# renmengye/rec-attend-public

Hardware: AMD Instinct MI355X
Metric: instance-timesteps/sec, full_model forward 512x512 T=16 (whole job; pipelined throughput: 8 batches in flight per GPU, fill and drain of the pipeline inside the timed region; config.lone_batch_* = one sync-bracketed forward) (higher is better)
Workload: dtype f32; 1 GPU; cfg2: CVPPP-arch full_model eval forward, 512x512, T=16, B=8 per GPU, y_out+s_out; arch=cvppp, H=512, W=512, T=16, batch_per_gpu=8, global_batch=8, parallelism=batch-sharded x1, no collective, ranks_in_communicator=1, hip_graph=True, tile_tickets=False, batches_in_flight=8, pipeline_slots=4, batches_per_launch=2, input=resident in HBM, output=left in HBM

## Files before the change

### rec-attend-public_amd/csrc/ra_common.h

```cpp
#pragma once
#include <hip/hip_runtime.h>

#include <cstdarg>
#include <cstdio>
#include <cstdlib>

#include "recattend.h"

namespace ra {

void set_error(const char *fmt, ...);

inline hipStream_t as_stream(void *s) { return reinterpret_cast<hipStream_t>(s); }

inline int launch_status(const char *what) {
  hipError_t e = hipGetLastError();
  if (e != hipSuccess) {
    set_error("%s: %s", what, hipGetErrorString(e));
    return static_cast<int>(e);
  }
  return 0;
}

inline int fail(int code, const char *fmt, ...) {
  char buf[256];
  va_list ap;
  va_start(ap, fmt);
  vsnprintf(buf, sizeof(buf), fmt, ap);
  va_end(ap);
  set_error("%s", buf);
  return code;
}

constexpr int kWave = 64;

inline int env_int(const char *name, int dflt) {
  const char *e = getenv(name);
  return e ? atoi(e) : dflt;
}

struct [[maybe_unused]] MaxDynamicLds {
  template <typename K>
  MaxDynamicLds(K kern, size_t bytes) {
    (void)hipFuncSetAttribute(reinterpret_cast<const void *>(kern), hipFuncAttributeMaxDynamicSharedMemorySize, (int)bytes);
  }
};

inline int cu_count() {
  static const int n = [] {
    int dev = 0;
    hipDeviceProp_t prop;
    if (hipGetDevice(&dev) == hipSuccess && hipGetDeviceProperties(&prop, dev) == hipSuccess && prop.multiProcessorCount > 0)
      return (int)prop.multiProcessorCount;
    return 256;
  }();
  return n;
}
template <typename K>
int wgs_per_cu(K kern, size_t lds) {
  MaxDynamicLds{kern, lds};
  int n = 0;
  if (hipOccupancyMaxActiveBlocksPerMultiprocessor(&n, kern, 256, lds) != hipSuccess || n < 1) n = 1;
  return n;
}

int tail_prio(int kind = 4);
__device__ __forceinline__ void raise_prio(int p) {
  if (p >= 3) __builtin_amdgcn_s_setprio(3);
  else if (p == 2) __builtin_amdgcn_s_setprio(2);
  else if (p == 1) __builtin_amdgcn_s_setprio(1);
}

constexpr int kTicketPoolStride = 32;
constexpr int kTicketSlotWords = 8 * kTicketPoolStride;
constexpr int kTicketMinTilesPerWg = 3;
unsigned *take_ticket_slots(int n, int grid_x);
int xcc_census_ok();

__device__ __forceinline__ int xcc_id() {
  unsigned id;
  asm volatile("s_getreg_b32 %0, hwreg(HW_REG_XCC_ID)" : "=s"(id));
  return (int)(id & 7u);
}
__device__ __forceinline__ unsigned ticket_draw(unsigned *pool) {
  const __amdgpu_buffer_rsrc_t r = __builtin_amdgcn_make_buffer_rsrc(pool, 0, 4, 0x00020000);
  return (unsigned)__builtin_amdgcn_raw_ptr_buffer_atomic_add_i32(1, r, 0, 0, 1);
}
struct TicketWalk {
  unsigned *pool;
  int base, lim;
  int cur, nxt;
  unsigned pend;
  __device__ __forceinline__ int tile_of(unsigned t) const { return t < (unsigned)lim ? base + (int)t : -1; }
  unsigned t0, t1;
  __device__ __forceinline__ void issue(unsigned *slot, int ntiles) {
    const int x = xcc_id(), chunk = (ntiles + 7) >> 3;
    pool = slot + x * kTicketPoolStride;
    base = x * chunk;
    lim = base + chunk <= ntiles ? chunk : (ntiles > base ? ntiles - base : 0);
    t0 = t1 = 0;
    if (threadIdx.x == 0) {
      t0 = ticket_draw(pool);
      t1 = ticket_draw(pool);
    }
  }
  __device__ __forceinline__ void begin(volatile unsigned *sh) {
    if (threadIdx.x == 0) sh[1] = t0;
    __syncthreads();
    cur = tile_of(__builtin_amdgcn_readfirstlane(sh[1]));
    nxt = -1;
    pend = t1;
  }
  __device__ __forceinline__ void request() {
    if (threadIdx.x == 0) pend = ticket_draw(pool);
  }
  __device__ __forceinline__ void read_next(volatile unsigned *sh) { nxt = tile_of(__builtin_amdgcn_readfirstlane(sh[0])); }
  __device__ __forceinline__ void publish(volatile unsigned *sh) {
    if (threadIdx.x == 0) sh[0] = pend;
  }
  __device__ __forceinline__ void step() { cur = nxt; }
};

__host__ __device__ inline int ceil_div(int a, int b) { return (a + b - 1) / b; }
__host__ __device__ inline int round_up(int a, int b) { return ceil_div(a, b) * b; }

inline void plan_walk(int *plan, int ntiles, int grid, int xcd_map) {
  int lo = ntiles / grid, hi = ceil_div(ntiles, grid);
  if (xcd_map) {
    const int chunk = (ntiles + 7) >> 3, nwx = grid >> 3;
    lo = hi = 0;
    for (int x = 0; x < 8; ++x) {
      const int n = x * chunk >= ntiles ? 0 : (x * chunk + chunk < ntiles ? chunk : ntiles - x * chunk);
      lo = (x == 0 || n / nwx < lo) ? n / nwx : lo;
      hi = ceil_div(n, nwx) > hi ? ceil_div(n, nwx) : hi;
    }
  }
  plan[RA_PLAN_GRID] = grid, plan[RA_PLAN_NTILES] = ntiles, plan[RA_PLAN_XCD_MAP] = xcd_map;
  plan[RA_PLAN_TILES_MIN] = lo, plan[RA_PLAN_TILES_MAX] = hi;
}
inline bool plan_have_device() {
  int n = 0;
  return hipGetDeviceCount(&n) == hipSuccess && n > 0;
}

}
```

### rec-attend-public_amd/csrc/ra_conv_pair.hip

```cpp
#include <cstdlib>

#include "ra_common.h"
#include "ra_split3.h"

namespace ra {
namespace cpair {

struct PArgs {
  const float *src;
  float *y;
  const float *wpA, *scA, *shA, *wpB, *scB, *shB;
  int C0, Hs, Ws, H, W, ups;
  int CoutAP, CoutB, CoutBP, poolB, Ho, Wo, reluA, reluB;
  const float *plane;
  int plane_chan;
  int bytes0, bytes_p;
  const float *cache;
  int cache_rows, cache_gx, bytes_c;
  int bytes_y;
  int xcd_map;
  float *rider_dst;
  int rider_quads;
  float rider_val;
  unsigned *tickets;
};

template <int CINA, int CMID, int NCB, int GX, int GYB>
struct PGeo {
  static constexpr int NCA = (CMID + 15) / 16;
  static constexpr int TWB = 8 * GX, THB = 8 * GYB, PMB = GX * GYB;
  static constexpr int GXA = GX + 1, GRA = THB / 2 + 1, NGA = GXA * GRA;
  static constexpr int AW = 8 * GXA, AH = 2 * GRA;
  static constexpr int LWA = AW + 2, LHA = AH + 2;
  static constexpr int NCGA = CINA / 4, CKA = CINA < 16 ? CINA : 16, NCHA = CINA / CKA, NCGAC = CKA / 4;
  static constexpr int NCGB = CMID / 4, CKB = CMID < 16 ? CMID : 16, NCHB = CMID / CKB, NCGBC = CKB / 4;
  static constexpr int KSA = 9 * NCGAC, KSB = 9 * NCGBC;
  static constexpr int IN_FLOATS = LHA * LWA * CINA;
  static constexpr int MID_FLOATS = AH * AW * CMID;
  static constexpr int RA = 4;
  static constexpr int GPW = (NGA + 3) / 4;
  static constexpr int ROUNDS = (GPW + RA - 1) / RA;
};

template <int N>
struct vec_of {
  typedef float type __attribute__((ext_vector_type(N)));
};

template <int CINA, int CMID, int NCB, int GX, int GYB>
__global__ __launch_bounds__(256) void conv_pair_mfma(const PArgs a, int tiles_x, int tiles_y) {
  using G = PGeo<CINA, CMID, NCB, GX, GYB>;
  constexpr int NCA = G::NCA;
  extern __shared__ __attribute__((aligned(16))) float lds[];
  float *tin = lds;
  float *tmid = lds + G::IN_FLOATS;
  typedef typename vec_of<G::NCGAC>::type avecA;
  typedef typename vec_of<G::NCGBC>::type avecB;

  const int tid = threadIdx.x, lane = tid & 63;
  const int wave = __builtin_amdgcn_readfirstlane(tid >> 6);
  const int m = lane & 15, ksub = lane >> 4;
  const int q = m >> 2, dy = (m >> 1) & 1, dx = m & 1;
  const int co_lane = lane & 15, qo = lane >> 4;
  const int per = tiles_x * tiles_y;
  const int b = blockIdx.x / per;
  const int trem = blockIdx.x - b * per;
  const int ty0 = (trem / tiles_x) * G::THB, tx0 = (trem % tiles_x) * G::TWB;

  {
    const int sy0 = a.ups ? (ty0 >> 1) : ty0, sx0 = a.ups ? (tx0 >> 1) : tx0;
    const float *base = a.src + ((size_t)(b * a.Hs + sy0) * a.Ws + sx0) * a.C0;
    for (int e = tid; e < G::LHA * G::LWA; e += 256) {
      const int rr = e / G::LWA - 2, cc = e % G::LWA - 2;
      const int Y = ty0 + rr, X = tx0 + cc;
      bool ok = (Y >= 0) & (Y < a.H) & (X >= 0) & (X < a.W);
      int ys = rr, xs = cc;
      if (a.ups) {
        ok = ok & (rr & 1) & (cc & 1);
        ys = rr >> 1;
        xs = cc >> 1;
      }
      f32x4 v[G::NCGA];
#pragma unroll
      for (int cg = 0; cg < G::NCGA; ++cg) {
        v[cg] = f32x4{0.f, 0.f, 0.f, 0.f};
        if (ok) v[cg] = *reinterpret_cast<const f32x4 *>(base + (ys * a.Ws + xs) * a.C0 + 4 * cg);
      }
      if (a.plane && ok) {
        const float pv = a.plane[(size_t)(b * a.Hs + sy0 + ys) * a.Ws + sx0 + xs];
        const int pg = a.plane_chan >> 2, slot = a.plane_chan & 3;
#pragma unroll
        for (int cg = 0; cg < G::NCGA; ++cg) {
          v[cg].x = (cg == pg && slot == 0) ? pv : v[cg].x;
          v[cg].y = (cg == pg && slot == 1) ? pv : v[cg].y;
          v[cg].z = (cg == pg && slot == 2) ? pv : v[cg].z;
          v[cg].w = (cg == pg && slot == 3) ? pv : v[cg].w;
        }
      }
      float *rec = tin + e * CINA;
#pragma unroll
      for (int ks = 0; ks < 4; ++ks) {
        if constexpr (G::NCGA == 1) {
          rec[ks] = v[0][ks];
// ... 347 lines not shown
    const int wrow0 = ty0 + wave * 2 * GYB, lcol0 = tx0 + 2 * qo;
#pragma unroll
    for (int n = 0; n < NCB; ++n) {
      const int co = 16 * n + co_lane;
      const float sc = a.scB[co], sh = a.shB[co];
      const bool co_ok = co < a.CoutB;
      const int obase = ((b * a.Ho + wrow0 / opool) * a.Wo + lcol0 / opool) * a.CoutB + co;
#pragma unroll
      for (int g = 0; g < G::PMB; ++g) {
        const int gx = g % GX, gy = g / GX;
        const int row0 = wrow0 + 2 * gy, col0 = lcol0 + 8 * gx;
        float v[4];
#pragma unroll
        for (int r = 0; r < 4; ++r) v[r] = fmaxf(acc[g][n][r] * sc + sh, loB);
        if (opool == 2) {
          const float o = fmaxf(fmaxf(v[0], v[1]), fmaxf(v[2], v[3]));
          if (co_ok && (row0 >> 1) < a.Ho && (col0 >> 1) < a.Wo)
            a.y[obase + (gy * a.Wo + 4 * gx) * a.CoutB] = o;
        } else {
#pragma unroll
          for (int r = 0; r < 4; ++r)
            if (co_ok && row0 + (r >> 1) < a.Ho && col0 + (r & 1) < a.Wo)
              a.y[obase + ((2 * gy + (r >> 1)) * a.Wo + 8 * gx + (r & 1)) * a.CoutB] = v[r];
        }
      }
    }
  }
  }
}

template <int CINA>
struct NGeo {
  static constexpr int TH = 16, TW = 32;
  static constexpr int NCGA = CINA / 4;
  static constexpr int AGX = 5, AGY = 5, NGA = AGX * AGY, GPW = (NGA + 3) / 4;
  static constexpr int AW = 41, AHS = TH + 2;
  static constexpr int LW = 43, LH = 4 * AGY + 2;
  static constexpr int LHL = TH + 4, LWL = TW + 6;
  static constexpr int IN_FLOATS = LH * LW * CINA;
  static constexpr int MID_FLOATS = AHS * AW * 8;
};

#ifndef RA_PAIR8_CACHE_AHEAD
#define RA_PAIR8_CACHE_AHEAD 0
#endif
#ifndef RA_PAIR8_OCC
#define RA_PAIR8_OCC 3
#endif
#ifdef RA_PROBE8
__device__ long long *ra_probe8_buf;
#define RA_PHASE_PROBE_BUF ra_probe8_buf
#define RA_PHASE_PROBE_WG blockIdx.x
#endif
#include "ra_phase_probe.h"
#ifdef RA_P8_NOBAR
#define RA_P8_SYNC() __builtin_amdgcn_s_waitcnt(0xc07f)
#else
#define RA_P8_SYNC() __syncthreads()
#endif
template <int CINA, bool CACHED, bool SPLIT = false>
__global__ __launch_bounds__(256, CACHED ? (SPLIT ? (RA_PAIR8_CACHE_AHEAD ? 2 : 3) : 4) : RA_PAIR8_OCC) void conv_pair8_mfma(const PArgs a, int tiles_x, int tiles_y, int ntiles) {
  using G = NGeo<CINA>;
  constexpr int NCGA = G::NCGA;
  static_assert(!CACHED || CINA == 4, "cached form: 4 input channels");
  static_assert(!SPLIT || CACHED, "the split-precision layer B exists for the cached (steady-state) form");
  constexpr int PLANE_B = G::AHS * G::AW * 16;
  constexpr int MIDF = SPLIT ? 3 * PLANE_B / 4 : G::MID_FLOATS;
  constexpr int RECA = CACHED ? 1 : CINA;
  extern __shared__ __attribute__((aligned(16))) float lds[];
  constexpr int IN_FLOATS = (G::LH * G::LW * RECA + 3) & ~3;
  float *tin = lds;
  float *tmid = lds + IN_FLOATS;
  typedef typename vec_of<NCGA>::type avecA;

  const int tid = threadIdx.x, lane = tid & 63;
  __shared__ unsigned tk_sh[2];
  TicketWalk tk;
  const bool dyn = a.tickets != nullptr;
  if (dyn) tk.issue(a.tickets, ntiles);
  const int wave = __builtin_amdgcn_readfirstlane(tid >> 6);
  const int m = lane & 15, ksub = lane >> 4;
  const int n = lane & 15, qo = lane >> 4;
  const int p = n >> 3, co = n & 7;
  const int per = tiles_x * tiles_y;

  const float scA = a.scA[co], scB = a.scB[co], shB = a.shB[co];
  const float loA = a.reluA ? 0.f : -__builtin_inff(), loB = a.reluB ? 0.f : -__builtin_inff();
  const int qA = m >> 2, rA = m & 3, pA = ksub >> 1, coA0 = 4 * (ksub & 1);
  f32x4 scA4, shA4;
#pragma unroll
  for (int j = 0; j < 4; ++j) scA4[j] = a.scA[coA0 + j], shA4[j] = a.shA[coA0 + j];
  const bool fill = !CACHED && a.cache != nullptr;
  float bA[CACHED ? 1 : 12][NCGA], bB[12][2];
  float bAc[3];
#pragma unroll
  for (int ky = 0; ky < 3; ++ky) {
    const int kx = ksub - p;
    const bool ok = (kx >= 0) & (kx <= 2);
    const int tap = ok ? ky * 3 + kx : 0;
    const float w = a.wpA[((tap * NCGA + (a.plane_chan >> 2)) * 4 + (a.plane_chan & 3)) * a.CoutAP + co];
    bAc[ky] = (CACHED && ok) ? w * scA : 0.f;
  }
#pragma unroll
  for (int ky = 0; ky < 3; ++ky)
#pragma unroll
    for (int kxp = 0; kxp < 4; ++kxp) {
      const int kx = kxp - p;
      const bool ok = (kx >= 0) & (kx <= 2);
      const int tap = ok ? ky * 3 + kx : 0;
      if constexpr (!CACHED) {
#pragma unroll
        for (int cg = 0; cg < NCGA; ++cg) {
          const float w = a.wpA[((tap * NCGA + cg) * 4 + ksub) * a.CoutAP + co];
          bA[ky * 4 + kxp][cg] = ok ? w * (fill ? 1.f : scA) : 0.f;
        }
      }
#pragma unroll
      for (int cg = 0; cg < 2; ++cg) {
        const float w = a.wpB[((tap * 2 + cg) * 4 + ksub) * a.CoutBP + co];
        bB[ky * 4 + kxp][cg] = ok ? w * scB : 0.f;
      }
    }

  s16x8 wB[SPLIT ? 3 : 1][SPLIT ? 3 : 1];
  if constexpr (SPLIT) {
#pragma unroll
    for (int ky = 0; ky < 3; ++ky) {
      const int kx = ksub - p;
      const bool ok = (kx >= 0) & (kx <= 2);
      const int tap = ok ? ky * 3 + kx : 0;
#pragma unroll
      for (int j = 0; j < 8; j += 2) {
        const float w0 = a.wpB[((tap * 2 + (j >> 2)) * 4 + (j & 3)) * a.CoutBP + co];
        const float w1 = a.wpB[((tap * 2 + ((j + 1) >> 2)) * 4 + ((j + 1) & 3)) * a.CoutBP + co];
        unsigned H, M, L;
        split3_pair(ok ? w0 * scB : 0.f, ok ? w1 * scB : 0.f, H, M, L);
        wB[ky][0][j] = (short)(H & 0xffffu), wB[ky][0][j + 1] = (short)(H >> 16);
        wB[ky][1][j] = (short)(M & 0xffffu), wB[ky][1][j + 1] = (short)(M >> 16);
        wB[ky][2][j] = (short)(L & 0xffffu), wB[ky][2][j + 1] = (short)(L >> 16);
      }
    }
  }
  const __amdgpu_buffer_rsrc_t rs = __builtin_amdgcn_make_buffer_rsrc(const_cast<float *>(a.src), 0, a.bytes0, 0x00020000);
  const __amdgpu_buffer_rsrc_t rp = __builtin_amdgcn_make_buffer_rsrc(
      const_cast<float *>(a.plane ? a.plane : a.src), 0, a.plane ? a.bytes_p : 0, 0x00020000);
  constexpr int NE = G::LHL * G::LWL, NIT = (NE + 255) / 256;
  int e_rr[NIT], e_cc[NIT];
#pragma unroll
  for (int i = 0; i < NIT; ++i) {
    const int e = tid + 256 * i;
    e_rr[i] = e / G::LWL;
    e_cc[i] = e - e_rr[i] * G::LWL;
    if (e >= NE) e_rr[i] = -(1 << 20);
  }
  unsigned e_offp[NIT], e_offs[NIT];
#pragma unroll
  for (int i = 0; i < NIT; ++i) {
    const bool in = tid + 256 * i < NE;
    const unsigned o = (unsigned)(e_rr[i] * a.W + e_cc[i]) * 4u;
    e_offp[i] = in ? o : 0x80000000u;
    e_offs[i] = in ? o * CINA : 0x80000000u;
  }
  struct TC {
    int b, ty, tx;
  };
  auto split = [&](int t) {
    TC c;
    c.b = t / per;
    const int r = t - c.b * per;
    c.ty = r / tiles_x;
    c.tx = r - c.ty * tiles_x;
    return c;
  };
  const int nwx = a.xcd_map ? (int)gridDim.x >> 3 : (int)gridDim.x;
  const int chunk = (ntiles + 7) >> 3;
  const int t_first = a.xcd_map ? ((int)blockIdx.x & 7) * chunk + ((int)blockIdx.x >> 3) : (int)blockIdx.x;
  const int t_end = a.xcd_map ? (((int)blockIdx.x & 7) * chunk + chunk < ntiles ? ((int)blockIdx.x & 7) * chunk + chunk : ntiles) : ntiles;
  const TC stride = split(nwx);
  auto advance = [&](TC c) {
    c.tx += stride.tx;
    if (c.tx >= tiles_x) {
      c.tx -= tiles_x;
      ++c.ty;
    }
    c.ty += stride.ty;
    if (c.ty >= tiles_y) {
      c.ty -= tiles_y;
      ++c.b;
    }
    c.b += stride.b;
    return c;
  };
  f32x4 v[NIT][NCGA];
  float pv[NIT];
  auto fetch = [&](const TC &c) {
    const int fb = c.b, fy0 = c.ty * G::TH - 2, fx0 = c.tx * G::TW - 3;
    const bool inside = (fy0 >= 0) & (fy0 + G::LHL <= a.H) & (fx0 >= 0) & (fx0 + G::LWL <= a.W);
    if (inside) {
      const unsigned base = (unsigned)((fb * a.H + fy0) * a.W + fx0) * 4u;
#pragma unroll
      for (int i = 0; i < NIT; ++i) {
        if constexpr (!CACHED) {
#pragma unroll
          for (int cg = 0; cg < NCGA; ++cg)
            v[i][cg] = __builtin_bit_cast(
                f32x4, __builtin_amdgcn_raw_buffer_load_b128(rs, (int)(base * CINA + e_offs[i] + 16u * cg), 0, 0));
        }
        pv[i] = __builtin_bit_cast(float, __builtin_amdgcn_raw_buffer_load_b32(rp, (int)(base + e_offp[i]), 0, 0));
      }
      return;
    }
#pragma unroll
    for (int i = 0; i < NIT; ++i) {
      const int Y = fy0 + e_rr[i], X = fx0 + e_cc[i];
      const bool ok = (Y >= 0) & (Y < a.H) & (X >= 0) & (X < a.W);
      const int pix = (fb * a.H + Y) * a.W + X;
      if constexpr (!CACHED) {
#pragma unroll
        for (int cg = 0; cg < NCGA; ++cg)
          v[i][cg] = __builtin_bit_cast(
              f32x4, __builtin_amdgcn_raw_buffer_load_b128(rs, ok ? (pix * CINA + 4 * cg) * 4 : 0x7fffffff, 0, 0));
      }
      pv[i] = __builtin_bit_cast(float, __builtin_amdgcn_raw_buffer_load_b32(rp, ok ? pix * 4 : 0x7fffffff, 0, 0));
    }
  };

  const int lane_in = CACHED ? (m >> 2) * G::LW + 2 * (m & 3) + ksub
                             : ((m >> 2) * G::LW + 2 * (m & 3)) * CINA + ksub * NCGA;
  const __amdgpu_buffer_rsrc_t rc = __builtin_amdgcn_make_buffer_rsrc(
      const_cast<float *>(a.cache ? a.cache : a.src), 0, a.cache ? a.bytes_c : 0, 0x00020000);
  const int lane_b = ((m & 1) * G::AW + 2 * (m >> 1) + 1) * 8 + ksub * 2;
  const int pg = a.plane_chan >> 2, slot = a.plane_chan & 3;

  int slot_c[G::GPW];
#pragma unroll
  for (int s = 0; s < G::GPW; ++s) {
    int gi = wave + 4 * s;
    if (gi >= G::NGA) gi = G::NGA - 1;
    const int gr = gi / G::AGX, gc = gi - gr * G::AGX;
    slot_c[s] = (4 * gr * a.cache_gx + gc) * 256;
  }
  const int lane_c = qA * a.cache_gx * 256 + rA * 64 + ksub * 16;
  const __amdgpu_buffer_rsrc_t ry = __builtin_amdgcn_make_buffer_rsrc(a.y, 0, a.bytes_y, 0x00020000);
  const unsigned lane_y = co < a.CoutB ? (unsigned)(((2 * qo + p) * a.CoutB + co) * 4) : 0x80000000u;
  int g_y[4];
#pragma unroll
  for (int g = 0; g < 4; ++g) g_y[g] = ((g >> 1) * a.Wo + 8 * (g & 1)) * a.CoutB * 4;

  int tile = t_first;
  if (dyn) {
    tk.begin(tk_sh);
    tile = tk.cur;
  }
  bool have = dyn ? tile >= 0 : tile < t_end;
  TC cur = split(have ? tile : 0), nxt = cur;
  if (have) fetch(cur);
  RA_PHASE_DECL;
  for (int e = tid; e < (IN_FLOATS + MIDF) / 4; e += 256)
    reinterpret_cast<f32x4 *>(lds)[e] = f32x4{0.f, 0.f, 0.f, 0.f};
  __syncthreads();
  const bool rider = !CACHED && a.rider_dst != nullptr;
  const __amdgpu_buffer_rsrc_t rr = __builtin_amdgcn_make_buffer_rsrc(rider ? a.rider_dst : a.y, 0,
                                                                       rider ? a.rider_quads * 16 : 0, 0x00020000);
  const int r_chunk = rider ? (a.rider_quads + (int)gridDim.x - 1) / (int)gridDim.x : 0;
  int r_idx = (int)blockIdx.x * r_chunk + tid;
  const int r_end = ((int)blockIdx.x + 1) * r_chunk < a.rider_quads ? ((int)blockIdx.x + 1) * r_chunk : a.rider_quads;
  const int my_tiles = t_end > t_first ? (t_end - t_first + nwx - 1) / nwx : 1;
  const int r_per_tile = (r_chunk + 256 * my_tiles - 1) / (256 * my_tiles);
  const u32x4 r_bits = __builtin_bit_cast(u32x4, f32x4{a.rider_val, a.rider_val, a.rider_val, a.rider_val});
  bool have_n = false;
  f32x4 cpre[CACHED ? G::GPW : 1];
  auto load_cache = [&](const TC &tc) {
    const int tile_c0 = ((tc.b * a.cache_rows + tc.ty * G::TH) * a.cache_gx + ((tc.tx * G::TW) >> 3)) * 256;
#pragma unroll
    for (int s = 0; s < (CACHED ? G::GPW : 1); ++s)
      cpre[s] = __builtin_bit_cast(f32x4, __builtin_amdgcn_raw_buffer_load_b128(rc, tile_c0 + slot_c[s] + lane_c, 0, 0));
  };
#if RA_PAIR8_CACHE_AHEAD
  if constexpr (CACHED) {
    if (have) load_cache(cur);
  }
#endif
  for (; have; tile = dyn ? (tk.step(), tk.cur) : tile + nwx, cur = nxt, have = have_n) {
    const int b = cur.b, ty0 = cur.ty * G::TH, tx0 = cur.tx * G::TW;
#if !RA_PAIR8_CACHE_AHEAD
    if constexpr (CACHED) load_cache(cur);
#endif

#pragma unroll
    for (int i = 0; i < NIT; ++i) {
      if constexpr (CACHED) {
        if (e_rr[i] >= 0) tin[e_rr[i] * G::LW + e_cc[i]] = pv[i];
        continue;
      }
      if (a.plane) {
#pragma unroll
        for (int cg = 0; cg < NCGA; ++cg) {
          v[i][cg].x = (cg == pg && slot == 0) ? pv[i] : v[i][cg].x;
          v[i][cg].y = (cg == pg && slot == 1) ? pv[i] : v[i][cg].y;
          v[i][cg].z = (cg == pg && slot == 2) ? pv[i] : v[i][cg].z;
          v[i][cg].w = (cg == pg && slot == 3) ? pv[i] : v[i][cg].w;
        }
      }
      if (e_rr[i] >= 0) {
        float *rec = tin + (e_rr[i] * G::LW + e_cc[i]) * CINA;
        if constexpr (NCGA == 1) {
          *reinterpret_cast<f32x4 *>(rec) = v[i][0];
        } else {
#pragma unroll
          for (int ks = 0; ks < 4; ++ks)
#pragma unroll
            for (int cg = 0; cg < NCGA; ++cg) rec[ks * NCGA + cg] = v[i][cg][ks];
        }
      }
    }
    if (dyn) tk.publish(tk_sh);
    RA_P8_SYNC();
    RA_PHASE_AT(0);
    if (dyn) {
      tk.read_next(tk_sh);
      tk.request();
      have_n = tk.nxt >= 0;
      nxt = split(have_n ? tk.nxt : 0);
    } else {
      have_n = tile + nwx < t_end;
      nxt = advance(cur);
    }
    if (have_n) fetch(nxt);
    if constexpr (!CACHED) {
      if (rider)
        for (int u = 0; u < r_per_tile; ++u, r_idx += 256)
          __builtin_amdgcn_raw_buffer_store_b128(r_bits, rr, r_idx < r_end ? r_idx * 16 : 0x7fffffff, 0, 0);
    }

    {
      const bool interior = (ty0 >= 1) & (ty0 + G::TH + 1 <= a.H) & (tx0 >= 2) & (tx0 + G::TW + 1 <= a.W);
      const int tile_c = ((b * a.cache_rows + ty0) * a.cache_gx + (tx0 >> 3)) * 256;
      f32x4 acc[G::GPW];
      int gin[G::GPW];
#pragma unroll
      for (int s = 0; s < G::GPW; ++s) {
        int gi = wave + 4 * s;
        if (gi >= G::NGA) gi = G::NGA - 1;
        const int gr = gi / G::AGX, gc = gi - gr * G::AGX;
        gin[s] = (4 * gr * G::LW + 8 * gc) * RECA + lane_in;
        if constexpr (CACHED) {
          acc[s] = cpre[s] * scA4 + shA4;
        } else {
          acc[s] = fill ? f32x4{0.f, 0.f, 0.f, 0.f} : shA4;
        }
      }
      RA_PHASE_AT(1);
      if constexpr (CACHED) {
#pragma unroll
        for (int ky = 0; ky < 3; ++ky) {
          float av[G::GPW];
#pragma unroll
          for (int s = 0; s < G::GPW; ++s) av[s] = tin[gin[s] + ky * G::LW];
#pragma unroll
          for (int s = 0; s < G::GPW; ++s)
            acc[s] = __builtin_amdgcn_mfma_f32_16x16x4f32(bAc[ky], av[s], acc[s], 0, 0, 0);
        }
      } else {
#pragma unroll
      for (int ky = 0; ky < 3; ++ky)
#pragma unroll
        for (int kxp = 0; kxp < 4; ++kxp) {
          avecA av[G::GPW];
#pragma unroll
          for (int s = 0; s < G::GPW; ++s)
            av[s] = *reinterpret_cast<const avecA *>(&tin[gin[s] + (ky * G::LW + kxp) * CINA]);
#pragma unroll
          for (int cg = 0; cg < NCGA; ++cg)
#pragma unroll
            for (int s = 0; s < G::GPW; ++s)
              acc[s] = __builtin_amdgcn_mfma_f32_16x16x4f32(bA[ky * 4 + kxp][cg], av[s][cg], acc[s], 0, 0, 0);
        }
      }
      if (fill) {
#pragma unroll
        for (int s = 0; s < G::GPW; ++s) {
          int gi = wave + 4 * s;
          if (gi >= G::NGA) gi = G::NGA - 1;
          const int gr = gi / G::AGX, gc = gi - gr * G::AGX;
          const bool mine = (4 * gr + qA < G::AHS) & ((gc < 4) | (tx0 + G::TW >= a.W));
          const int off = mine ? tile_c + slot_c[s] + lane_c : 0x7fffffff;
          __builtin_amdgcn_raw_buffer_store_b128(__builtin_bit_cast(__attribute__((ext_vector_type(4))) unsigned, acc[s]), rc, off, 0, 0);
          acc[s] = acc[s] * scA4 + shA4;
        }
      }
#pragma unroll
      for (int s = 0; s < G::GPW; ++s) {
        const int gi = wave + 4 * s;
        const int gr = gi / G::AGX, gc = gi - gr * G::AGX;
        const bool live = (gi < G::NGA) & (4 * gr + qA < G::AHS);
        float o[4];
#pragma unroll
        for (int j = 0; j < 4; ++j) o[j] = fmaxf(acc[s][j], loA);
        if (!interior) {
          const int Y = ty0 - 1 + 4 * gr + qA, X = tx0 - 2 + 8 * gc + 2 * rA + pA;
          const bool ok = (Y >= 0) & (Y < a.H) & (X >= 0) & (X < a.W);
#pragma unroll
          for (int j = 0; j < 4; ++j) o[j] = ok ? o[j] : 0.f;
        }
        const int pix = (4 * gr + qA) * G::AW + 8 * gc + 2 * rA + pA;
        if constexpr (SPLIT) {
          unsigned H01, M01, L01, H23, M23, L23;
          split3_pair(o[0], o[1], H01, M01, L01);
          split3_pair(o[2], o[3], H23, M23, L23);
          if (live) {
            unsigned char *d0 = reinterpret_cast<unsigned char *>(tmid) + pix * 16 + coA0 * 2;
            *reinterpret_cast<u32x2 *>(d0) = u32x2{H01, H23};
            *reinterpret_cast<u32x2 *>(d0 + PLANE_B) = u32x2{M01, M23};
            *reinterpret_cast<u32x2 *>(d0 + 2 * PLANE_B) = u32x2{L01, L23};
          }
        } else if (live) {
          float *dst = tmid + pix * 8 + (ksub & 1);
#pragma unroll
          for (int j = 0; j < 4; ++j) dst[2 * j] = o[j];
        }
      }
    }
    RA_PHASE_AT(2);
    RA_P8_SYNC();
    RA_PHASE_AT(3);

#if RA_PAIR8_CACHE_AHEAD
    if constexpr (CACHED) {
      if (have_n) load_cache(nxt);
    }
#endif
    {
      f32x4 acc[4];
      int gmid[4];
#pragma unroll
      for (int g = 0; g < 4; ++g) {
        const int gy = 2 * wave + (g >> 1), gx = g & 1;
        gmid[g] = (2 * gy * G::AW + 16 * gx) * 8 + lane_b;
        acc[g] = f32x4{shB, shB, shB, shB};
      }
      if constexpr (SPLIT) {
        const unsigned char *tb = reinterpret_cast<const unsigned char *>(tmid);
        const int lane_px = ((m & 1) * G::AW + 2 * (m >> 1) + 1 + ksub) * 16;
#pragma unroll
        for (int ky = 0; ky < 3; ++ky)
#pragma unroll
          for (int gh = 0; gh < 2; ++gh) {
            s16x8 av[2][3];
#pragma unroll
            for (int u = 0; u < 2; ++u) {
              const int g = 2 * gh + u;
              const int gy = 2 * wave + (g >> 1), gx = g & 1;
              const int off = ((2 * gy + ky) * G::AW + 16 * gx) * 16 + lane_px;
#pragma unroll
              for (int pc = 0; pc < 3; ++pc) av[u][pc] = *reinterpret_cast<const s16x8 *>(tb + off + pc * PLANE_B);
            }
            constexpr int PA[6] = {1, 0, 2, 0, 1, 0}, PB[6] = {1, 2, 0, 1, 0, 0};
#pragma unroll
            for (int t = 0; t < 6; ++t)
#pragma unroll
              for (int u = 0; u < 2; ++u)
                acc[2 * gh + u] = __builtin_amdgcn_mfma_f32_16x16x32_bf16(__builtin_bit_cast(bf16x8, av[u][PA[t]]),
                                                                          __builtin_bit_cast(bf16x8, wB[ky][PB[t]]), acc[2 * gh + u], 0, 0, 0);
          }
      } else {
#pragma unroll
      for (int ky = 0; ky < 3; ++ky)
#pragma unroll
        for (int kxp = 0; kxp < 4; ++kxp) {
          f32x2 av[4];
#pragma unroll
          for (int g = 0; g < 4; ++g)
            av[g] = *reinterpret_cast<const f32x2 *>(&tmid[gmid[g] + (ky * G::AW + kxp) * 8]);
#pragma unroll
          for (int cg = 0; cg < 2; ++cg)
#pragma unroll
            for (int g = 0; g < 4; ++g)
              acc[g] = __builtin_amdgcn_mfma_f32_16x16x4f32(av[g][cg], bB[ky * 4 + kxp][cg], acc[g], 0, 0, 0);
        }
      }
      const int prow0 = (ty0 >> 1) + wave * 2, pcol0 = (tx0 >> 1) + 2 * qo + p;
      const bool whole = ((ty0 >> 1) + G::TH / 2 <= a.Ho) & ((tx0 >> 1) + G::TW / 2 <= a.Wo);
      const unsigned tile_y = (unsigned)(((b * a.Ho + prow0) * a.Wo + (tx0 >> 1)) * a.CoutB * 4) + lane_y;
#pragma unroll
      for (int g = 0; g < 4; ++g) {
        const float t0 = fmaxf(fmaxf(acc[g][0], acc[g][1]), loB), t1 = fmaxf(fmaxf(acc[g][2], acc[g][3]), loB);
        const float u0 = fmaxf(t0, __builtin_bit_cast(float, __builtin_amdgcn_mov_dpp(__builtin_bit_cast(int, t0), 0x128, 0xf, 0xf, true)));
        const float u1 = fmaxf(t1, __builtin_bit_cast(float, __builtin_amdgcn_mov_dpp(__builtin_bit_cast(int, t1), 0x128, 0xf, 0xf, true)));
        const float ov = p ? u1 : u0;
        const int prow = prow0 + (g >> 1), pcol = pcol0 + 8 * (g & 1);
        unsigned off = tile_y + (unsigned)g_y[g];
        if (!whole) off = ((prow < a.Ho) & (pcol < a.Wo)) ? off : 0x80000000u;
        __builtin_amdgcn_raw_buffer_store_b32(__builtin_bit_cast(unsigned, ov), ry, (int)off, 0, 0);
      }
    }
    RA_PHASE_AT(4);
  }
  RA_PHASE_END;
  if constexpr (!CACHED) {
    if (rider)
      for (; r_idx < r_end; r_idx += 256) __builtin_amdgcn_raw_buffer_store_b128(r_bits, rr, r_idx * 16, 0, 0);
  }
}

template <int CINA, bool CACHED = false, bool SPLIT = false>
int launch8(const PArgs &a_in, int B, hipStream_t st, int *plan) {
  using G = NGeo<CINA>;
  PArgs a = a_in;
  a.bytes_y = (int)((size_t)B * a.Ho * a.Wo * a.CoutB * sizeof(float));
  auto kern = conv_pair8_mfma<CINA, CACHED, SPLIT>;
  constexpr size_t lds = (size_t)(((G::LH * G::LW * (CACHED ? 1 : CINA) + 3) & ~3) + (SPLIT ? 3 * G::AHS * G::AW * 4 : G::MID_FLOATS)) * sizeof(float);
  const int tiles_x = ceil_div(a.W, G::TW), tiles_y = ceil_div(a.H, G::TH);
  const int ntiles = tiles_x * tiles_y * B;
  static const int wgs = env_int("RA_PAIR8_WGS", 768);
  static const int xcd = env_int("RA_PAIR8_XCD", 1);
  PArgs a2 = a;
  const int grid = ntiles < wgs ? ntiles : wgs;
  a2.xcd_map = (xcd && grid % 8 == 0 && grid >= 8) ? 1 : 0;
  const bool draws = CACHED && ntiles >= kTicketMinTilesPerWg * grid;
  if (plan) {
    plan[RA_PLAN_FAMILY] = RA_PLAN_FAMILY_PAIR;
    plan[RA_PLAN_FORM] = RA_PLAN_FORM_NPACKED | (CACHED ? RA_PLAN_FORM_CACHED : 0) | (SPLIT ? RA_PLAN_FORM_SPLIT : 0);
    plan[RA_PLAN_CK] = CINA, plan[RA_PLAN_CMID] = 8, plan[RA_PLAN_KF] = 3, plan[RA_PLAN_TILE_H] = G::TH, plan[RA_PLAN_TILE_W] = G::TW;
    plan[RA_PLAN_TILES_X] = tiles_x, plan[RA_PLAN_TILES_Y] = tiles_y, plan[RA_PLAN_TICKETS] = draws ? 1 : 0;
    plan_walk(plan, ntiles, grid, a2.xcd_map);
    return 0;
  }
  static const MaxDynamicLds lds_limit(kern, lds);
  a2.tickets = draws ? take_ticket_slots(1, grid) : nullptr;
  hipLaunchKernelGGL(kern, dim3(grid), dim3(256), lds, st, a2, tiles_x, tiles_y, ntiles);
  return launch_status("ra_conv_pair_f32");
}

__global__ __launch_bounds__(256) void first_cache_kernel(const float *x, const float *wpA, int CoutAP, int plane_chan,
                                                          int B, int H, int W, int rows, int ngx, float *cache) {
  __shared__ float sm[4][64][9];
  const int xl = threadIdx.x & 63, yl = threadIdx.x >> 6;
  const int X = blockIdx.x * 64 - 2 + xl, Y = blockIdx.y * 4 + yl, b = blockIdx.z;
  float acc[8];
#pragma unroll
  for (int co = 0; co < 8; ++co) acc[co] = 0.f;
  if (X >= 0 && X < W && Y < H) {
#pragma unroll
    for (int ky = 0; ky < 3; ++ky) {
      const int yy = Y + ky - 1;
#pragma unroll
      for (int kx = 0; kx < 3; ++kx) {
        const int xx = X + kx - 1;
        const bool ok = (yy >= 0) & (yy < H) & (xx >= 0) & (xx < W);
        f32x4 v = f32x4{0.f, 0.f, 0.f, 0.f};
        if (ok) v = *reinterpret_cast<const f32x4 *>(x + ((size_t)(b * H + yy) * W + xx) * 4);
        const float *wt = wpA + (size_t)((ky * 3 + kx) * 4) * CoutAP;
#pragma unroll
        for (int ci = 0; ci < 4; ++ci) {
          const float xv = ci == plane_chan ? 0.f : v[ci];
#pragma unroll
          for (int co = 0; co < 8; ++co) acc[co] = fmaf(xv, wt[ci * CoutAP + co], acc[co]);
        }
      }
    }
  }
#pragma unroll
  for (int co = 0; co < 8; ++co) sm[yl][xl][co] = acc[co];
  __syncthreads();
  for (int e = threadIdx.x; e < 4 * 8 * 16; e += 256) {
    const int n4 = e & 3, r = (e >> 2) & 3, g = (e >> 4) & 7, row = e >> 7;
    const int p = n4 >> 1, co0 = 4 * (n4 & 1);
    const int Yo = blockIdx.y * 4 + row, gx = blockIdx.x * 8 + g;
    if (Yo < H && gx < ngx) {
      f32x4 o;
#pragma unroll
      for (int j = 0; j < 4; ++j) o[j] = sm[row][8 * g + 2 * r + p][co0 + j];
      *reinterpret_cast<f32x4 *>(cache + (((size_t)b * rows + (Yo + 1)) * ngx + gx) * 64 + r * 16 + 4 * n4) = o;
    }
  }
}

inline void cache_dims(int H, int W, int &rows, int &ngx) {
  rows = ceil_div(H, NGeo<4>::TH) * NGeo<4>::TH + 4;
  ngx = ceil_div(W, NGeo<4>::TW) * (NGeo<4>::TW / 8) + 1;
}

template <int CINA, int CMID, int NCB, int GX, int GYB>
int launch(const PArgs &a, int B, hipStream_t st, int *plan) {
  using G = PGeo<CINA, CMID, NCB, GX, GYB>;
  auto kern = conv_pair_mfma<CINA, CMID, NCB, GX, GYB>;
  constexpr size_t lds = (size_t)(G::IN_FLOATS + G::MID_FLOATS) * sizeof(float);
  static_assert(lds <= 160 * 1024, "pair tile does not fit LDS");
  const int tiles_x = ceil_div(a.W, G::TWB), tiles_y = ceil_div(a.H, G::THB);
  const int ntiles = tiles_x * tiles_y * B;
  if (plan) {
    plan[RA_PLAN_FAMILY] = RA_PLAN_FAMILY_PAIR;
    plan[RA_PLAN_CK] = CINA, plan[RA_PLAN_CMID] = CMID, plan[RA_PLAN_NC] = NCB, plan[RA_PLAN_GX] = GX, plan[RA_PLAN_GY] = GYB;
    plan[RA_PLAN_KF] = 3, plan[RA_PLAN_TILE_H] = G::THB, plan[RA_PLAN_TILE_W] = G::TWB;
    plan[RA_PLAN_TILES_X] = tiles_x, plan[RA_PLAN_TILES_Y] = tiles_y, plan[RA_PLAN_NTILES] = ntiles;
    plan[RA_PLAN_GRID] = ntiles, plan[RA_PLAN_TILES_MIN] = plan[RA_PLAN_TILES_MAX] = 1;
    if (!(G::NCHA == 1 && G::NCHB == 1) || a.ups || a.plane) return 0;
    if (!plan_have_device()) {
      plan[RA_PLAN_GRID] = plan[RA_PLAN_TILES_MIN] = plan[RA_PLAN_TILES_MAX] = -1;
      return 0;
    }
// ... 258 lines not shown
```

### rec-attend-public_amd/csrc/ra_conv_wino.hip

```cpp
#include "ra_common.h"
#include "ra_split3.h"

#ifndef RA_PAIRW_SPLIT_OCC
#define RA_PAIRW_SPLIT_OCC 3
#endif
namespace ra {
namespace wino {


constexpr int TS = 16;
constexpr int WS = TS + 2;
constexpr int TEX = 36;

struct WArgs {
  const float *x, *wp, *scale, *shift;
  float *y;
  int B, H, W, Cout, relu;
  int bytes_x;
  int xcd_map;
  unsigned *tickets;
};

struct TileWalk {
  int first, end, step;
// ... 397 lines not shown
      }
      }
      RA_PHASE_AT(2);
#pragma unroll
      for (int s = 0; s < GPW; ++s) {
        const int g = p + 4 * s;
        if (g < NGA) {
          const int li = 16 * g + m;
          f32x4 o = acc[s] * scA4 + shA4;
#pragma unroll
          for (int j = 0; j < 4; ++j) o[j] = fmaxf(o[j], loA);
          if (!interior) {
            const int wr = li / WS, wc = li - wr * WS;
            const int Y = oyA + wr, X = oxA + wc;
            const bool ok = (Y >= 0) & (Y < a.H) & (X >= 0) & (X < a.W);
#pragma unroll
            for (int j = 0; j < 4; ++j) o[j] = ok ? o[j] : 0.f;
          }
          float *d = tin + li * S + 4 * ksub;
          *reinterpret_cast<f32x2 *>(d) = f32x2{o[0], o[1]};
          *reinterpret_cast<f32x2 *>(d + 2) = f32x2{o[2], o[3]};
        }
      }
    }
    RA_PHASE_AT(3);
    __syncthreads();
    RA_PHASE_AT(4);

#pragma unroll 1
    for (int mblk = 0; mblk < NMB; ++mblk) {
      const int tyi = 2 * mblk + (m >> 3), txi = m & 7;
      const float *pa = tin + ((2 * tyi + ra) * WS + 2 * txi) * S + ksub;
      const float *pb = tin + ((2 * tyi + rb) * WS + 2 * txi) * S + ksub;
      f32x4 acc[4];
#pragma unroll
      for (int q = 0; q < 4; ++q) acc[q] = f32x4{0.f, 0.f, 0.f, 0.f};
#pragma unroll
      for (int kk = 0; kk < KK; ++kk) {
        float r[4];
#pragma unroll
        for (int j = 0; j < 4; ++j) r[j] = pa[j * S + 4 * kk] + sg * pb[j * S + 4 * kk];
        const float v[4] = {r[0] - r[2], r[1] + r[2], r[2] - r[1], r[1] - r[3]};
#pragma unroll
        for (int q = 0; q < 4; ++q) acc[q] = __builtin_amdgcn_mfma_f32_16x16x4f32(bw[q][kk], v[q], acc[q], 0, 0, 0);
      }
      RA_PHASE_AT(5);
      if (mblk) __syncthreads();
      {
        const f32x4 t0 = acc[0] + acc[1] + acc[2];
        const f32x4 t1 = acc[1] - acc[2] - acc[3];
        *reinterpret_cast<f32x4 *>(&tex[((p * 2 + 0) * 16 + m) * TEXP + 4 * ksub]) = t0;
        *reinterpret_cast<f32x4 *>(&tex[((p * 2 + 1) * 16 + m) * TEXP + 4 * ksub]) = t1;
      }
      __syncthreads();
      {
        const int tl = tid >> 4;
        float T[4][2];
#pragma unroll
        for (int pp = 0; pp < 4; ++pp)
#pragma unroll
          for (int j = 0; j < 2; ++j) T[pp][j] = tex[((pp * 2 + j) * 16 + tl) * TEXP + eco];
        float best = -__builtin_inff();
#pragma unroll
        for (int j = 0; j < 2; ++j) {
          best = fmaxf(best, fmaxf((T[0][j] + T[1][j] + T[2][j]) * scB + shB, loB));
          best = fmaxf(best, fmaxf((T[1][j] - T[2][j] - T[3][j]) * scB + shB, loB));
        }
        const int oty = ty * (TSY / 2) + 2 * mblk + (tl >> 3), otx = tx * 8 + (tl & 7);
        a.y[((size_t)(b * Ho + oty) * Wo + otx) * 16 + eco] = best;
      }
      RA_PHASE_AT(6);
    }
  }
  RA_PHASE_END;
}

template <int TSY, bool SPLIT = false>
int launch_pair(const PWArgs &a, hipStream_t st, int *plan) {
  auto kern = conv_pair_wino_mfma<TSY, SPLIT>;
  constexpr int inf = SPLIT ? 3 * (TSY + 4) * (TS + 4) * 4 : (TSY + 4) * (TS + 4) * 8;
  constexpr int r0 = inf > 8 * 16 * 20 ? inf : 8 * 16 * 20;
  constexpr size_t lds = (size_t)(r0 + ((TSY + 2) * WS + 16) * 18) * sizeof(float);
  static const int resident = wgs_per_cu(kern, lds) * cu_count();
  static const int wgs = env_int("RA_PAIRW_WGS", 0);
  static const int cap = wgs > 0 ? wgs : resident;
  const int tiles_x = a.W / TS, tiles_y = a.H / TSY, ntiles = tiles_x * tiles_y * a.B;
  static const int xcd = env_int("RA_PAIRW_XCD", 1);
  const int grid = ntiles < cap ? ntiles : cap;
  PWArgs a2 = a;
  a2.xcd_map = (xcd && grid % 8 == 0 && grid >= 8) ? 1 : 0;
  const bool draws = ntiles >= 2 * kTicketMinTilesPerWg * grid;
  if (plan) {
    plan[RA_PLAN_FAMILY] = RA_PLAN_FAMILY_PAIR_WINO, plan[RA_PLAN_FORM] = SPLIT ? RA_PLAN_FORM_SPLIT : 0;
    plan[RA_PLAN_CK] = 8, plan[RA_PLAN_CMID] = 16, plan[RA_PLAN_NC] = 1, plan[RA_PLAN_KF] = 3, plan[RA_PLAN_POOL] = 2, plan[RA_PLAN_SLICES] = 1;
    plan[RA_PLAN_TILE_H] = TSY, plan[RA_PLAN_TILE_W] = TS, plan[RA_PLAN_TILES_X] = tiles_x, plan[RA_PLAN_TILES_Y] = tiles_y;
    plan[RA_PLAN_TICKETS] = draws ? 1 : 0;
    plan_walk(plan, ntiles, grid, a2.xcd_map);
    return 0;
  }
  a2.tickets = draws ? take_ticket_slots(1, grid) : nullptr;
  hipLaunchKernelGGL(kern, dim3(grid), dim3(256), lds, st, a2, tiles_x, tiles_y, ntiles);
  return launch_status("ra_conv_pair_wino_f32");
}

}
}

using namespace ra;

extern "C" int ra_conv_wino_supported(int Cin, int Cout, int pool, int H, int W) {
  return (Cin == 16 || Cin == 32) && Cout > 0 && Cout % 16 == 0 && (pool == 1 || pool == 2) && H > 0 && W > 0 &&
         H % wino::TS == 0 && W % wino::TS == 0;
}

extern "C" size_t ra_conv_wino_packed_floats(int Cin, int Cout) {
  if (!(Cin == 16 || Cin == 32) || Cout <= 0 || Cout % 16) return 0;
  return (size_t)16 * Cin * Cout;
}

extern "C" int ra_conv_wino_pack_weights(const float *w, int Cin, int Cout, float *out) {
  if (!w || !out || !ra_conv_wino_packed_floats(Cin, Cout)) return fail(RA_E_SHAPE, "ra_conv_wino_pack_weights: Cin %d Cout %d", Cin, Cout);
  static const float G[4][3] = {{1.f, 0.f, 0.f}, {0.5f, 0.5f, 0.5f}, {0.5f, -0.5f, 0.5f}, {0.f, 0.f, 1.f}};
  const int KK = Cin / 4, NBT = Cout / 16;
  for (int p = 0; p < 4; ++p)
    for (int q = 0; q < 4; ++q)
      for (int ci = 0; ci < Cin; ++ci)
        for (int co = 0; co < Cout; ++co) {
          double u = 0.0;
          for (int ky = 0; ky < 3; ++ky)
            for (int kx = 0; kx < 3; ++kx) u += (double)G[p][ky] * (double)G[q][kx] * (double)w[((size_t)(ky * 3 + kx) * Cin + ci) * Cout + co];
          const int kk = ci / 4, ks = ci % 4, nb = co / 16, n = co % 16;
          out[((size_t)((p * 4 + q) * KK + kk) * NBT + nb) * 64 + ks * 16 + n] = (float)u;
        }
  return 0;
}

static int wino_entry(const float *x, int B, int H, int W, int Cin, const float *wpacked, const float *scale, const float *shift, int Cout,
                      int relu, int pool, float *y, void *stream, int *plan) {
  if ((!plan && (!x || !wpacked || !scale || !shift || !y)) || B <= 0) return fail(RA_E_INVALID, "ra_conv_wino_f32: bad argument");
  if (!ra_conv_wino_supported(Cin, Cout, pool, H, W))
    return fail(RA_E_SHAPE, "ra_conv_wino_f32: Cin=%d Cout=%d pool=%d %dx%d", Cin, Cout, pool, H, W);
  const size_t bytes = (size_t)B * H * W * Cin * sizeof(float);
  if (bytes >= (1ull << 31)) return fail(RA_E_SHAPE, "ra_conv_wino_f32: input exceeds 2 GiB");
  wino::WArgs a{};
  a.x = x;
  a.wp = wpacked;
  a.scale = scale;
  a.shift = shift;
  a.y = y;
  a.B = B;
  a.H = H;
  a.W = W;
  a.Cout = Cout;
  a.relu = relu;
  a.bytes_x = (int)bytes;
  a.xcd_map = 0;
  hipStream_t st = as_stream(stream);
  if (Cout % 32) {
    if (Cin == 16) return pool == 2 ? wino::launch_any<16, 2, 1>(a, st, plan) : wino::launch_any<16, 1, 1>(a, st, plan);
    return pool == 2 ? wino::launch_any<32, 2, 1>(a, st, plan) : wino::launch_any<32, 1, 1>(a, st, plan);
  }
  if (Cin == 16) return pool == 2 ? wino::launch_any<16, 2, 2>(a, st, plan) : wino::launch_any<16, 1, 2>(a, st, plan);
  return pool == 2 ? wino::launch_any<32, 2, 2>(a, st, plan) : wino::launch_any<32, 1, 2>(a, st, plan);
}

extern "C" int ra_conv_wino_f32(const float *x, int B, int H, int W, int Cin, const float *wpacked, const float *scale,
                                const float *shift, int Cout, int relu, int pool, float *y, void *stream) {
  return wino_entry(x, B, H, W, Cin, wpacked, scale, shift, Cout, relu, pool, y, stream, nullptr);
// ... 56 lines not shown
```

Measured before the change: 57440 instance-timesteps/s.

## Walk pair-conv tiles in contiguous column runs and carry overlap rows

```diff
diff --git a/rec-attend-public_amd/csrc/ra_common.h b/rec-attend-public_amd/csrc/ra_common.h
--- a/rec-attend-public_amd/csrc/ra_common.h
+++ b/rec-attend-public_amd/csrc/ra_common.h
@@ -5,6 +5,7 @@
 #include <cstdio>
 #include <cstdlib>
 
+#include "ra_tile_walk.h"
 #include "recattend.h"
 
 namespace ra {
@@ -121,23 +122,6 @@
   __device__ __forceinline__ void step() { cur = nxt; }
 };
 
-__host__ __device__ inline int ceil_div(int a, int b) { return (a + b - 1) / b; }
-__host__ __device__ inline int round_up(int a, int b) { return ceil_div(a, b) * b; }
-
-inline void plan_walk(int *plan, int ntiles, int grid, int xcd_map) {
-  int lo = ntiles / grid, hi = ceil_div(ntiles, grid);
-  if (xcd_map) {
-    const int chunk = (ntiles + 7) >> 3, nwx = grid >> 3;
-    lo = hi = 0;
-    for (int x = 0; x < 8; ++x) {
-      const int n = x * chunk >= ntiles ? 0 : (x * chunk + chunk < ntiles ? chunk : ntiles - x * chunk);
-      lo = (x == 0 || n / nwx < lo) ? n / nwx : lo;
-      hi = ceil_div(n, nwx) > hi ? ceil_div(n, nwx) : hi;
-    }
-  }
-  plan[RA_PLAN_GRID] = grid, plan[RA_PLAN_NTILES] = ntiles, plan[RA_PLAN_XCD_MAP] = xcd_map;
-  plan[RA_PLAN_TILES_MIN] = lo, plan[RA_PLAN_TILES_MAX] = hi;
-}
 inline bool plan_have_device() {
   int n = 0;
   return hipGetDeviceCount(&n) == hipSuccess && n > 0;
diff --git a/rec-attend-public_amd/csrc/ra_conv_pair.hip b/rec-attend-public_amd/csrc/ra_conv_pair.hip
--- a/rec-attend-public_amd/csrc/ra_conv_pair.hip
+++ b/rec-attend-public_amd/csrc/ra_conv_pair.hip
@@ -19,6 +19,7 @@
   int cache_rows, cache_gx, bytes_c;
   int bytes_y;
   int xcd_map;
+  int carry;
   float *rider_dst;
   int rider_quads;
   float rider_val;
@@ -532,7 +533,6 @@
   const int m = lane & 15, ksub = lane >> 4;
   const int n = lane & 15, qo = lane >> 4;
   const int p = n >> 3, co = n & 7;
-  const int per = tiles_x * tiles_y;
 
   const float scA = a.scA[co], scB = a.scB[co], shB = a.shB[co];
   const float loA = a.reluA ? 0.f : -__builtin_inff(), loB = a.reluB ? 0.f : -__builtin_inff();
@@ -611,36 +611,13 @@
     e_offp[i] = in ? o : 0x80000000u;
     e_offs[i] = in ? o * CINA : 0x80000000u;
   }
-  struct TC {
-    int b, ty, tx;
-  };
-  auto split = [&](int t) {
-    TC c;
-    c.b = t / per;
-    const int r = t - c.b * per;
-    c.ty = r / tiles_x;
-    c.tx = r - c.ty * tiles_x;
-    return c;
-  };
-  const int nwx = a.xcd_map ? (int)gridDim.x >> 3 : (int)gridDim.x;
-  const int chunk = (ntiles + 7) >> 3;
-  const int t_first = a.xcd_map ? ((int)blockIdx.x & 7) * chunk + ((int)blockIdx.x >> 3) : (int)blockIdx.x;
-  const int t_end = a.xcd_map ? (((int)blockIdx.x & 7) * chunk + chunk < ntiles ? ((int)blockIdx.x & 7) * chunk + chunk : ntiles) : ntiles;
-  const TC stride = split(nwx);
-  auto advance = [&](TC c) {
-    c.tx += stride.tx;
-    if (c.tx >= tiles_x) {
-      c.tx -= tiles_x;
-      ++c.ty;
-    }
-    c.ty += stride.ty;
-    if (c.ty >= tiles_y) {
-      c.ty -= tiles_y;
-      ++c.b;
-    }
-    c.b += stride.b;
-    return c;
-  };
+  using TC = TileCoord;
+  auto split = [&](int t) { return column_tile(t, tiles_x, tiles_y); };
+  const TileRun run = column_run(ntiles, (int)gridDim.x, (int)blockIdx.x, a.xcd_map);
+  const int t_first = run.first, t_end = run.end;
+  constexpr bool CARRY_FORM = CACHED && SPLIT;
+  constexpr int GPC = CARRY_FORM ? G::AGX : G::GPW;
+  static_assert(!CARRY_FORM || (G::AGY == 5 && G::AHS == 18), "carried tile: group rows 0..3, shifted down by two rows");
   f32x4 v[NIT][NCGA];
   float pv[NIT];
   auto fetch = [&](const TC &c) {
@@ -715,26 +692,27 @@
   const int r_chunk = rider ? (a.rider_quads + (int)gridDim.x - 1) / (int)gridDim.x : 0;
   int r_idx = (int)blockIdx.x * r_chunk + tid;
   const int r_end = ((int)blockIdx.x + 1) * r_chunk < a.rider_quads ? ((int)blockIdx.x + 1) * r_chunk : a.rider_quads;
-  const int my_tiles = t_end > t_first ? (t_end - t_first + nwx - 1) / nwx : 1;
+  const int my_tiles = t_end > t_first ? t_end - t_first : 1;
   const int r_per_tile = (r_chunk + 256 * my_tiles - 1) / (256 * my_tiles);
   const u32x4 r_bits = __builtin_bit_cast(u32x4, f32x4{a.rider_val, a.rider_val, a.rider_val, a.rider_val});
   bool have_n = false;
   f32x4 cpre[CACHED ? G::GPW : 1];
-  auto load_cache = [&](const TC &tc) {
-    const int tile_c0 = ((tc.b * a.cache_rows + tc.ty * G::TH) * a.cache_gx + ((tc.tx * G::TW) >> 3)) * 256;
+  auto load_cache = [&](const TC &tc, bool cy) {
+    const int tile_c0 = ((tc.b * a.cache_rows + tc.ty * G::TH + (cy ? 2 : 0)) * a.cache_gx + ((tc.tx * G::TW) >> 3)) * 256;
 #pragma unroll
     for (int s = 0; s < (CACHED ? G::GPW : 1); ++s)
-      cpre[s] = __builtin_bit_cast(f32x4, __builtin_amdgcn_raw_buffer_load_b128(rc, tile_c0 + slot_c[s] + lane_c, 0, 0));
+      if (s < GPC || !cy) cpre[s] = __builtin_bit_cast(f32x4, __builtin_amdgcn_raw_buffer_load_b128(rc, tile_c0 + slot_c[s] + lane_c, 0, 0));
   };
 #if RA_PAIR8_CACHE_AHEAD
   if constexpr (CACHED) {
-    if (have) load_cache(cur);
+    if (have) load_cache(cur, false);
   }
 #endif
-  for (; have; tile = dyn ? (tk.step(), tk.cur) : tile + nwx, cur = nxt, have = have_n) {
+  bool carry = false, carry_n = false;
+  for (; have; tile = dyn ? (tk.step(), tk.cur) : tile + 1, cur = nxt, have = have_n, carry = carry_n) {
     const int b = cur.b, ty0 = cur.ty * G::TH, tx0 = cur.tx * G::TW;
 #if !RA_PAIR8_CACHE_AHEAD
-    if constexpr (CACHED) load_cache(cur);
+    if constexpr (CACHED) load_cache(cur, carry);
 #endif
 
 #pragma unroll
@@ -773,9 +751,10 @@
       have_n = tk.nxt >= 0;
       nxt = split(have_n ? tk.nxt : 0);
     } else {
-      have_n = tile + nwx < t_end;
-      nxt = advance(cur);
-    }
+      have_n = tile + 1 < t_end;
+      nxt = column_next(cur, tiles_x, tiles_y);
+    }
+    if constexpr (CARRY_FORM) carry_n = a.carry && have_n && (!dyn || tk.nxt == tile + 1) && nxt.ty != 0;
     if (have_n) fetch(nxt);
     if constexpr (!CACHED) {
       if (rider)
@@ -786,6 +765,7 @@
     {
       const bool interior = (ty0 >= 1) & (ty0 + G::TH + 1 <= a.H) & (tx0 >= 2) & (tx0 + G::TW + 1 <= a.W);
       const int tile_c = ((b * a.cache_rows + ty0) * a.cache_gx + (tx0 >> 3)) * 256;
+      const int dr = carry ? 2 : 0;
       f32x4 acc[G::GPW];
       int gin[G::GPW];
 #pragma unroll
@@ -793,9 +773,9 @@
         int gi = wave + 4 * s;
         if (gi >= G::NGA) gi = G::NGA - 1;
         const int gr = gi / G::AGX, gc = gi - gr * G::AGX;
-        gin[s] = (4 * gr * G::LW + 8 * gc) * RECA + lane_in;
+        gin[s] = ((4 * gr + dr) * G::LW + 8 * gc) * RECA + lane_in;
         if constexpr (CACHED) {
-          acc[s] = cpre[s] * scA4 + shA4;
+          acc[s] = (s < GPC || !carry) ? cpre[s] * scA4 + shA4 : f32x4{0.f, 0.f, 0.f, 0.f};
         } else {
           acc[s] = fill ? f32x4{0.f, 0.f, 0.f, 0.f} : shA4;
         }
@@ -804,12 +784,25 @@
       if constexpr (CACHED) {
 #pragma unroll
         for (int ky = 0; ky < 3; ++ky) {
-          float av[G::GPW];
-#pragma unroll
-          for (int s = 0; s < G::GPW; ++s) av[s] = tin[gin[s] + ky * G::LW];
-#pragma unroll
-          for (int s = 0; s < G::GPW; ++s)
+          float av[GPC];
+#pragma unroll
+          for (int s = 0; s < GPC; ++s) av[s] = tin[gin[s] + ky * G::LW];
+#pragma unroll
+          for (int s = 0; s < GPC; ++s)
             acc[s] = __builtin_amdgcn_mfma_f32_16x16x4f32(bAc[ky], av[s], acc[s], 0, 0, 0);
+        }
+        if constexpr (GPC < G::GPW) {
+          if (!carry) {
+#pragma unroll
+            for (int ky = 0; ky < 3; ++ky) {
+              float av[G::GPW - GPC];
+#pragma unroll
+              for (int s = GPC; s < G::GPW; ++s) av[s - GPC] = tin[gin[s] + ky * G::LW];
+#pragma unroll
+              for (int s = GPC; s < G::GPW; ++s)
+                acc[s] = __builtin_amdgcn_mfma_f32_16x16x4f32(bAc[ky], av[s - GPC], acc[s], 0, 0, 0);
+            }
+          }
         }
       } else {
 #pragma unroll
@@ -839,21 +832,36 @@
           acc[s] = acc[s] * scA4 + shA4;
         }
       }
+      if constexpr (CARRY_FORM) {
+        if (carry) {
+#pragma unroll
+          for (int s = (3 * G::AGX) / 4; s < GPC; ++s) {
+            const int gi = wave + 4 * s;
+            const int gr = gi / G::AGX, gc = gi - gr * G::AGX;
+            if (gr == 3 && lane < 48) {
+              const int pc = lane >> 4, px = (lane & 15) >> 3, cx = lane & 7;
+              unsigned char *row0 = reinterpret_cast<unsigned char *>(tmid) + pc * PLANE_B + (px * G::AW + 8 * gc + cx) * 16;
+              *reinterpret_cast<u32x4 *>(row0) = *reinterpret_cast<const u32x4 *>(row0 + G::TH * G::AW * 16);
+            }
+          }
+        }
+      }
 #pragma unroll
       for (int s = 0; s < G::GPW; ++s) {
+        if (s >= GPC && carry) continue;
         const int gi = wave + 4 * s;
         const int gr = gi / G::AGX, gc = gi - gr * G::AGX;
-        const bool live = (gi < G::NGA) & (4 * gr + qA < G::AHS);
+        const bool live = (gi < G::NGA) & (4 * gr + dr + qA < G::AHS);
         float o[4];
 #pragma unroll
         for (int j = 0; j < 4; ++j) o[j] = fmaxf(acc[s][j], loA);
         if (!interior) {
-          const int Y = ty0 - 1 + 4 * gr + qA, X = tx0 - 2 + 8 * gc + 2 * rA + pA;
+          const int Y = ty0 - 1 + 4 * gr + dr + qA, X = tx0 - 2 + 8 * gc + 2 * rA + pA;
           const bool ok = (Y >= 0) & (Y < a.H) & (X >= 0) & (X < a.W);
 #pragma unroll
           for (int j = 0; j < 4; ++j) o[j] = ok ? o[j] : 0.f;
         }
-        const int pix = (4 * gr + qA) * G::AW + 8 * gc + 2 * rA + pA;
+        const int pix = (4 * gr + dr + qA) * G::AW + 8 * gc + 2 * rA + pA;
         if constexpr (SPLIT) {
           unsigned H01, M01, L01, H23, M23, L23;
           split3_pair(o[0], o[1], H01, M01, L01);
@@ -877,7 +885,7 @@
 
 #if RA_PAIR8_CACHE_AHEAD
     if constexpr (CACHED) {
-      if (have_n) load_cache(nxt);
+      if (have_n) load_cache(nxt, carry_n);
     }
 #endif
     {
@@ -962,11 +970,12 @@
   constexpr size_t lds = (size_t)(((G::LH * G::LW * (CACHED ? 1 : CINA) + 3) & ~3) + (SPLIT ? 3 * G::AHS * G::AW * 4 : G::MID_FLOATS)) * sizeof(float);
   const int tiles_x = ceil_div(a.W, G::TW), tiles_y = ceil_div(a.H, G::TH);
   const int ntiles = tiles_x * tiles_y * B;
-  static const int wgs = env_int("RA_PAIR8_WGS", 768);
+  const int wgs_env = env_int("RA_PAIR8_WGS", 768), wgs = wgs_env > 0 ? wgs_env : 768;
   static const int xcd = env_int("RA_PAIR8_XCD", 1);
   PArgs a2 = a;
   const int grid = ntiles < wgs ? ntiles : wgs;
   a2.xcd_map = (xcd && grid % 8 == 0 && grid >= 8) ? 1 : 0;
+  a2.carry = (CACHED && SPLIT && env_int("RA_PAIR_CARRY", 1) != 0) ? 1 : 0;
   const bool draws = CACHED && ntiles >= kTicketMinTilesPerWg * grid;
   if (plan) {
     plan[RA_PLAN_FAMILY] = RA_PLAN_FAMILY_PAIR;
diff --git a/rec-attend-public_amd/csrc/ra_conv_wino.hip b/rec-attend-public_amd/csrc/ra_conv_wino.hip
--- a/rec-attend-public_amd/csrc/ra_conv_wino.hip
+++ b/rec-attend-public_amd/csrc/ra_conv_wino.hip
@@ -503,8 +503,8 @@
   constexpr int r0 = inf > 8 * 16 * 20 ? inf : 8 * 16 * 20;
   constexpr size_t lds = (size_t)(r0 + ((TSY + 2) * WS + 16) * 18) * sizeof(float);
   static const int resident = wgs_per_cu(kern, lds) * cu_count();
-  static const int wgs = env_int("RA_PAIRW_WGS", 0);
-  static const int cap = wgs > 0 ? wgs : resident;
+  const int wgs = env_int("RA_PAIRW_WGS", 0);
+  const int cap = wgs > 0 ? wgs : resident;
   const int tiles_x = a.W / TS, tiles_y = a.H / TSY, ntiles = tiles_x * tiles_y * a.B;
   static const int xcd = env_int("RA_PAIRW_XCD", 1);
   const int grid = ntiles < cap ? ntiles : cap;
diff --git a/rec-attend-public_amd/csrc/ra_tile_walk.h b/rec-attend-public_amd/csrc/ra_tile_walk.h
--- /dev/null
+++ b/rec-attend-public_amd/csrc/ra_tile_walk.h
@@ -0,0 +1,67 @@
+#pragma once
+#include "recattend.h"
+
+#if defined(__HIPCC__) || defined(__CUDACC__)
+#define RA_HD __host__ __device__
+#else
+#define RA_HD
+#endif
+
+namespace ra {
+
+RA_HD inline int ceil_div(int a, int b) { return (a + b - 1) / b; }
+RA_HD inline int round_up(int a, int b) { return ceil_div(a, b) * b; }
+
+inline void plan_walk(int *plan, int ntiles, int grid, int xcd_map) {
+  int lo = ntiles / grid, hi = ceil_div(ntiles, grid);
+  if (xcd_map) {
+    const int chunk = (ntiles + 7) >> 3, nwx = grid >> 3;
+    lo = hi = 0;
+    for (int x = 0; x < 8; ++x) {
+      const int n = x * chunk >= ntiles ? 0 : (x * chunk + chunk < ntiles ? chunk : ntiles - x * chunk);
+      lo = (x == 0 || n / nwx < lo) ? n / nwx : lo;
+      hi = ceil_div(n, nwx) > hi ? ceil_div(n, nwx) : hi;
+    }
+  }
+  plan[RA_PLAN_GRID] = grid, plan[RA_PLAN_NTILES] = ntiles, plan[RA_PLAN_XCD_MAP] = xcd_map;
+  plan[RA_PLAN_TILES_MIN] = lo, plan[RA_PLAN_TILES_MAX] = hi;
+}
+
+struct TileRun {
+  int first, end;
+};
+RA_HD inline TileRun column_run(int ntiles, int grid, int g, int xcd_map) {
+  int base = 0, n = ntiles, w = g, nw = grid;
+  if (xcd_map) {
+    const int chunk = (ntiles + 7) >> 3, x = g & 7;
+    base = x * chunk < ntiles ? x * chunk : ntiles;
+    n = base + chunk < ntiles ? chunk : ntiles - base;
+    w = g >> 3, nw = grid >> 3;
+  }
+  const int q = n / nw, r = n - q * nw;
+  TileRun run;
+  run.first = base + w * q + (w < r ? w : r);
+  run.end = run.first + q + (w < r ? 1 : 0);
+  return run;
+}
+struct TileCoord {
+  int b, ty, tx;
+};
+RA_HD inline TileCoord column_tile(int t, int tiles_x, int tiles_y) {
+  TileCoord c;
+  const int per = tiles_x * tiles_y;
+  c.b = t / per;
+  const int r = t - c.b * per;
+  c.tx = r / tiles_y;
+  c.ty = r - c.tx * tiles_y;
+  return c;
+}
+RA_HD inline TileCoord column_next(TileCoord c, int tiles_x, int tiles_y) {
+  if (++c.ty >= tiles_y) {
+    c.ty = 0;
+    if (++c.tx >= tiles_x) c.tx = 0, ++c.b;
+  }
+  return c;
+}
+
+}
```

Result: no change. 57180 instance-timesteps/s (-0.5%).
